# 1812598631/Amos-slam

Measured on AMD Instinct MI355X. Metric: front-end frames/sec (ORB extract+match+mask) at 640x480, higher is better.
Workload: dtype u8 (ORB, gate, matcher) + fp32 (mask network); 1 GPU; configs[2]: 640x480 L8 N1000 full front-end: YOLACT-R50 fp32 mask + ORB detect + gate + describe + match; lanes_per_gpu=2, frames_per_launch=64, width=640, height=480, n_features=1000, n_levels=8, ini_th_fast=20, min_th_fast=7, match=frame k vs k-1, N x N best-2, synthetic_stream_seed=stream = rank, frame k seeded 1000*rank+k (amos-slam_amd/synth.py), parallelism=frames sharded 1 ways, one process per GPU, no data-path collective

## Files before the change

### amos-slam_amd/__init__.py

```python
import ctypes as C
import os

import numpy as np

_HERE = os.path.dirname(os.path.abspath(__file__))
LIB_PATH = os.environ.get("AMOS_FRONTEND_LIB", os.path.join(_HERE, "csrc", "libamos_frontend.so"))

KP_DTYPE = np.dtype([("x", "<f4"), ("y", "<f4"), ("size", "<f4"), ("angle", "<f4"),
                     ("response", "<f4"), ("octave", "<i4"), ("class_id", "<i4")])
BEST2_DTYPE = np.dtype([("best_idx", "<i4"), ("best_dist", "<i4"), ("second_idx", "<i4"),
                        ("second_dist", "<i4")])

TH_HIGH, TH_LOW, HISTO_LENGTH = 100, 50, 30

_v, _i, _z, _f, _d, _q, _u = C.c_void_p, C.c_int, C.c_size_t, C.c_float, C.c_double, C.c_longlong, C.c_uint32
PROTOTYPES = {
    "amos_last_error": (C.c_char_p, ()),
    "amos_device_count": (_i, ()),
    "amos_current_device": (_i, ()),
    "amos_build_variant": (C.c_char_p, ()),
    "amos_orb_create": (_i, (_v, _i, _i, _i, _i, _v, _v)),
    "amos_orb_destroy": (None, (_v,)),
    "amos_orb_geometry_probe": (_i, (_v, _i, _i, _i, _i, _v, _v)),
    "amos_orb_tables": (_i, (_v, _v, _v, _v, _v, _v, _v)),
# ... 53 lines not shown
    "amos_mask_bias_relu_maxpool_device": (_i, (_v, _v, _v, _v, _i, _i, _i, _i)),
    "amos_mask_stem_weight_floats": (_i, ()),
    "amos_mask_stem_weights_device": (_i, (_v, _v, _q, _q, _q, _q, _v)),
    "amos_mask_stem_device": (_i, (_v, _v, _q, _q, _q, _q, _v, _v, _v, _i, _i, _i)),
    "amos_mask_conv_supported": (_i, (_i, _i, _i, _i, _i, _i)),
    "amos_mask_conv_device": (_i, (_v, _v, _v, _v, _v, _v, _i, _i, _i, _i, _i, _i, _i, _i, _i, _i)),
    "amos_mask_conv_workspace_bytes": (_z, (_i, _i, _i, _i, _i, _i, _i, _i, _i)),
    "amos_mask_conv_ws_device": (_i, (_v, _v, _v, _v, _v, _v, _i, _i, _i, _i, _i, _i, _i, _i, _i, _i, _v, _z)),
    "amos_mask_conv_tile_mode": (_i, (_i,)),
    "amos_mask_conv_kernel_name": (_i, (_i, _i, _i, _i, _i, _i, _i, _i, _i, _v, _i)),
    "amos_mask_conv_chain_supported": (_i, (_i, _i, _i, _i, _i, _i, _i)),
    "amos_mask_conv_chain_device": (_i, (_v, _v, _v, _v, _v, _v, _v, _v, _i, _i, _i, _i, _i, _i, _i)),
    "amos_mask_conv1x1_supported": (_i, (_i, _i, _i)),
    "amos_mask_winograd_supported": (_i, (_i, _i)),
    "amos_mask_winograd_weight_floats": (_z, (_i, _i)),
    "amos_mask_winograd_weights_device": (_i, (_v, _v, _v, _i, _i)),
    "amos_mask_winograd_conv_device": (_i, (_v, _v, _v, _v, _v, _v, _i, _i, _i, _i, _i, _i)),
    "amos_mask_winograd24_weight_floats": (_z, (_i, _i)),
    "amos_mask_winograd24_weights_device": (_i, (_v, _v, _v, _i, _i)),
    "amos_mask_winograd24_conv_device": (_i, (_v, _v, _v, _v, _v, _v, _i, _i, _i, _i, _i, _i)),
    "amos_mask_winograd24_conv_layout_device": (_i, (_v, _v, _v, _v, _v, _v, _i, _i, _i, _i, _i, _i, _i, _i)),
    "amos_mask_winograd24_persistent_mode": (_i, (_i,)),
    "amos_mask_winograd24_narrow_mode": (_i, (_i,)),
    "amos_mask_conv1x1_device": (_i, (_v, _v, _v, _v, _v, _v, _i, _i, _i, _i, _i, _i, _i)),
    "amos_mask_bilinear_nhwc_device": (_i, (_v, _v, _v, _i, _i, _i, _i, _i, _i, _f, _f)),
    "amos_mask_bilinear_nhwc_act_device": (_i, (_v, _v, _v, _i, _i, _i, _i, _i, _i, _f, _f, _i)),
    "amos_mask_bilinear_x2_mode": (_i, (_i,)),
    "amos_mask_nms_column_max_device": (_i, (_v, _v, _v, _i, _i)),
    "amos_mask_class_scores_device": (_i, (_v, _v, _v, _i, _i, _i, _f)),
    "amos_mask_person_mask_device": (_i, (_v, _v, _v, _v, _i, _i, _i, _i, _i, _i)),
    "amos_mask_head_outputs_device": (_i, (_v, _v, _v, _v, _v, _v, _i, _i, _i, _i, _i, _i, _i, _i)),
    "amos_mask_head_outputs_scores_device": (_i, (_v, _v, _v, _v, _v, _v, _v, _f, _i, _i, _i, _i, _i, _i, _i, _i)),
    "amos_mask_topk_rows_device": (_i, (_v, _v, _v, _v, _i, _i, _i)),
    "amos_mask_topk_rows_sparse_device": (_i, (_v, _v, _v, _v, _i, _i, _i, _f)),
    "amos_mask_post_workspace_bytes": (_z, (_i, _i, _i, _i, _i, _i)),
    "amos_mask_person_masks_device": (_i, (_v, _v, _v, _v, _v, _v, _i, _i, _i, _i, _i, _i, _i, _i, _v, _z, _v, _v)),
    "amos_mask_person_masks_scores_device": (_i, (_v, _v, _v, _v, _v, _v, _i, _i, _i, _i, _i, _i, _i, _i, _v, _z, _v, _v)),
    "amos_slic_center_count": (_i, (_i, _i, _i, _v, _v)),
    "amos_slic_create": (_i, (_i, _v, _i, _i, _i, _v)),
    "amos_slic_destroy": (None, (_v,)),
    "amos_slic_stream": (_v, (_v,)),
    "amos_slic_run": (_i, (_v, _v, _v, _i, _i, _i, _i, _i, _v, _v, _v)),
    "amos_slic_batch_device": (_i, (_v, _v, _v, _i, _i, _i, _i, _i, _i, _v, _v)),
    "amos_cluster_bgr2lab_batch_device": (_i, (_v, _v, _z, _i, _v)),
    "amos_cluster_kmeans_batch_device": (_i, (_v, _v, _i, _i, _i, _u, _i, _v)),
    "amos_cluster_kmeans": (_i, (_v, _v, _i, _i, _u, _i, _v)),
# ... 432 lines not shown


def mask_conv_supported(cin, cout, kh, kw, stride, pad):
    return lib().amos_mask_conv_supported(cin, cout, kh, kw, stride, pad) == 0


def mask_winograd_supported(cin, cout):
    return lib().amos_mask_winograd_supported(cin, cout) == 0


def mask_winograd_weights(stream_ptr, w_ptr, u_ptr, cin, cout):
    _check(lib().amos_mask_winograd_weights_device(stream_ptr, w_ptr, u_ptr, cin, cout), "amos_mask_winograd_weights_device")


def mask_winograd_conv(stream_ptr, x_ptr, u_ptr, bias_ptr, residual_ptr, y_ptr, batch, h, w, cin, cout, relu):
    _check(lib().amos_mask_winograd_conv_device(stream_ptr, x_ptr, u_ptr, bias_ptr, residual_ptr, y_ptr, batch, h, w, cin, cout, int(relu)),
           "amos_mask_winograd_conv_device")


def mask_winograd24_weights(stream_ptr, w_ptr, u_ptr, cin, cout):
    _check(lib().amos_mask_winograd24_weights_device(stream_ptr, w_ptr, u_ptr, cin, cout), "amos_mask_winograd24_weights_device")


def mask_winograd24_conv(stream_ptr, x_ptr, u_ptr, bias_ptr, residual_ptr, y_ptr, batch, h, w, cin, cout, relu):
    _check(lib().amos_mask_winograd24_conv_device(stream_ptr, x_ptr, u_ptr, bias_ptr, residual_ptr, y_ptr, batch, h, w, cin, cout, int(relu)),
           "amos_mask_winograd24_conv_device")


def mask_winograd24_conv_layout(stream_ptr, x_ptr, u_ptr, bias_ptr, residual_ptr, y_ptr, batch, h, w, cin, cout, relu, in_blocked, out_blocked):
    _check(lib().amos_mask_winograd24_conv_layout_device(stream_ptr, x_ptr, u_ptr, bias_ptr, residual_ptr, y_ptr, batch, h, w, cin, cout, int(relu), int(in_blocked),
                                                         int(out_blocked)), "amos_mask_winograd24_conv_layout_device")


def mask_winograd24_persistent_mode(mode=-2):
    return int(lib().amos_mask_winograd24_persistent_mode(mode))


def mask_winograd24_narrow_mode(mode=-2):
    return int(lib().amos_mask_winograd24_narrow_mode(mode))


def mask_conv_tile_mode(mode=-2):
    return int(lib().amos_mask_conv_tile_mode(mode))


def mask_conv_kernel_name(batch, in_h, in_w, cin, cout, kh, kw, stride, pad):
    buf = C.create_string_buffer(96)
    _check(lib().amos_mask_conv_kernel_name(batch, in_h, in_w, cin, cout, kh, kw, stride, pad, buf, 96), "amos_mask_conv_kernel_name")
    return buf.value.decode()


def mask_conv(stream_ptr, x_ptr, w_ptr, bias_ptr, residual_ptr, y_ptr, batch, in_h, in_w, cin, cout, kh, kw, stride, pad, relu):
    _check(lib().amos_mask_conv_device(stream_ptr, x_ptr, w_ptr, bias_ptr, residual_ptr, y_ptr, batch, in_h, in_w, cin, cout, kh, kw, stride, pad, int(relu)),
           "amos_mask_conv_device")
# ... 318 lines not shown
```

### amos-slam_amd/csrc/amos_mask_post.hip

```cpp
#include <hip/hip_runtime.h>
#include <stdint.h>

#include "../../include/amos_frontend.h"
#include "amos_common.h"

namespace amos {

constexpr int kScoreTile = 64;
__global__ __launch_bounds__(256) void k_class_scores(const float *__restrict__ conf, float *__restrict__ scores, int P, int C1, float thresh)
{
    extern __shared__ float tile[];
    __shared__ float best[kScoreTile];
    const int b = blockIdx.y, p0 = blockIdx.x * kScoreTile, np = min(kScoreTile, P - p0), pitch = C1 + 1;
    const float *src = conf + ((size_t)b * P + p0) * C1;
    for (int e = threadIdx.x; e < np * C1; e += 256) {
        const int r = e / C1, c = e - r * C1;
        tile[r * pitch + c] = src[e];
    }
    __syncthreads();
    if (threadIdx.x < np) {
        const float *row = tile + threadIdx.x * pitch;
        float m = row[1];
        bool nan = m != m;
        for (int c = 2; c < C1; c++) {
// ... 61 lines not shown
            }
        } else {
            for (int i = 0; i < n; i++) {
                if (!flags[b * n + i]) continue;
                const float *m = masks + ((size_t)b * n + i) * ph * pw;
                const float p = m[y0 * pw + x0], r = m[y0 * pw + x1], s2 = m[y1 * pw + x0], u = m[y1 * pw + x1];
                const float v = __fadd_rn(__fmul_rn(hy, __fadd_rn(__fmul_rn(hx, p), __fmul_rn(lx, r))), __fmul_rn(ly, __fadd_rn(__fmul_rn(hx, s2), __fmul_rn(lx, u))));
                count += v > 0.5f ? 1u : 0u;
            }
        }
        out[((size_t)b * H + oy) * W + ox] = (uint8_t)((count * 255u) & 0xffu);
    }
}

constexpr int kHeadCells = 16;
__global__ __launch_bounds__(256) void k_head_outputs(const float *__restrict__ raw, const float *__restrict__ bias, float *__restrict__ loc, float *__restrict__ conf,
                                                     float *__restrict__ coef, int cells, int cpad, int A, int C1, int D, int P, int pOff,
                                                     float *__restrict__ scores, float thresh)
{
    extern __shared__ float sh[];
    const int b = blockIdx.y, c0 = blockIdx.x * kHeadCells, nc = min(kHeadCells, cells - c0);
    const int nLoc = A * 4, nConf = A * C1, nCoef = A * D;
    const float *src = raw + ((size_t)b * cells + c0) * cpad;
    for (int e = threadIdx.x * 4; e < nc * cpad; e += 256 * 4) {
        float4 v = *reinterpret_cast<const float4 *>(src + e);
        const float4 bb = *reinterpret_cast<const float4 *>(bias + e % cpad);
        v.x = __fadd_rn(v.x, bb.x); v.y = __fadd_rn(v.y, bb.y); v.z = __fadd_rn(v.z, bb.z); v.w = __fadd_rn(v.w, bb.w);
        *reinterpret_cast<float4 *>(sh + e) = v;
    }
    __syncthreads();
    __shared__ float sMax[256], sSum[256];
#define AMOS_HEAD_FOREACH(n, body)                                                             \
    {                                                                                          \
        const int stepCell = 256 / (n), stepR = 256 % (n);                                     \
        int cell = (int)threadIdx.x / (n), r = (int)threadIdx.x - cell * (n);                  \
        for (int e = threadIdx.x; e < nc * (n); e += 256) {                                    \
            body;                                                                              \
            cell += stepCell;                                                                  \
            r += stepR;                                                                        \
            if (r >= (n)) { r -= (n); cell++; }                                                \
        }                                                                                      \
    }
    if ((int)threadIdx.x < nc * A) {
        const int cell = threadIdx.x / A, a = threadIdx.x - cell * A;
        const float *v = sh + cell * cpad + nLoc + a * C1;
        float m = v[0];
        for (int c = 1; c < C1; c++) m = fmaxf(m, v[c]);
// ... 852 lines not shown
```

### amos-slam_amd/csrc/amos_winograd24.hip

```cpp
#include <hip/hip_runtime.h>
#include <stdint.h>
#include <stdio.h>
#include <stdlib.h>

#include <algorithm>

#include "../../include/amos_frontend.h"
#include "amos_common.h"

namespace amos {

constexpr int kW24Tiles = 32;
constexpr int kW24Cout = 64;
constexpr int kW24K = 8;
constexpr int kW24Threads = 512;
constexpr int kW24Pos = 24;
#ifndef AMOS_W24_GROUP
#define AMOS_W24_GROUP 16
#endif
constexpr int kW24Group = AMOS_W24_GROUP;
constexpr int kW24StageU = kW24Pos * kW24Cout * kW24K;
constexpr int kW24PosV = kW24Tiles * kW24K;
constexpr int kW24StageV = kW24Pos * kW24PosV;
constexpr int kW24RawCols = 256;
constexpr int kW24RawRow = kW24RawCols * kW24K;
constexpr int kW24StageR = 4 * kW24RawRow;
#ifndef AMOS_W24_XAHEAD
#define AMOS_W24_XAHEAD 1
#endif
constexpr int kW24RawBufs = AMOS_W24_XAHEAD + 1;
constexpr int kW24ExchangeFloats = 8 * 4 * 32 * 32;
constexpr int kW24LoopFloats = 2 * kW24StageV + kW24RawBufs * kW24StageR;
constexpr int kW24LdsFloats = kW24ExchangeFloats > kW24LoopFloats ? kW24ExchangeFloats : kW24LoopFloats;

typedef float f32x16 __attribute__((ext_vector_type(16)));
typedef float f32x4 __attribute__((ext_vector_type(4)));

struct W24Args {
    const float *x, *u, *bias, *res;
    float *y;
    int B, H, W, C, N;
    int tilesX, tilesY, tilesPerImage, totalTiles;
    int mBlocks, nTiles, stages, relu;
    unsigned xBytes;
    unsigned xPixelBytes, xStageBytes;
    int outBlocked;
    int virtualBlocks;
};

__device__ __forceinline__ f32x4 w24_fma(float k, f32x4 a, f32x4 b)
{
    return f32x4{__builtin_fmaf(k, a.x, b.x), __builtin_fmaf(k, a.y, b.y), __builtin_fmaf(k, a.z, b.z), __builtin_fmaf(k, a.w, b.w)};
}

__device__ __host__ __forceinline__ int w24_swz(int row, int half) { return row * 8 + 4 * (half ^ (((row >> 2) ^ (row >> 3)) & 1)); }
__device__ __forceinline__ int w24_raw_unit(int col, int quad) { return (col >> 5) * 64 + (col & 3) * 16 + ((col & 31) >> 2) * 2 + quad; }

__global__ __launch_bounds__(256) void k_winograd24_weights(const float *__restrict__ w, float *__restrict__ u, int cin, int cout)
{
    const int idx = blockIdx.x * 256 + threadIdx.x;
    if (idx >= cin * cout) return;
    const int c = idx % cin, n = idx / cin;
    double g[3][3];
    for (int a = 0; a < 3; a++)
        for (int b = 0; b < 3; b++) g[a][b] = (double)w[((size_t)(n * 3 + a) * 3 + b) * cin + c];
    double t[4][3];
    for (int b = 0; b < 3; b++) {
        t[0][b] = g[0][b];
        t[1][b] = 0.5 * (g[0][b] + g[1][b] + g[2][b]);
        t[2][b] = 0.5 * (g[0][b] - g[1][b] + g[2][b]);
        t[3][b] = g[2][b];
    }
    const int stages = cin / kW24K, nt = n / kW24Cout, nr = n % kW24Cout, s = c / kW24K, k = c % kW24K;
    float *img = u + (size_t)(nt * stages + s) * kW24StageU + (size_t)((nr >> 5) * 64 + (k >> 2) * 32 + (nr & 31)) * 4 + (k & 3);
    for (int a = 0; a < 4; a++) {
        const double t0 = t[a][0], t1 = t[a][1], t2 = t[a][2];
        const double r[6] = {t0 / 4.0, -(t0 + t1 + t2) / 6.0, -(t0 - t1 + t2) / 6.0, t0 / 24.0 + t1 / 12.0 + t2 / 6.0, t0 / 24.0 - t1 / 12.0 + t2 / 6.0, t2};
        for (int b = 0; b < 6; b++) img[(size_t)(a * 6 + b) * 512] = (float)r[b];
    }
}

template <int kHalf, bool kPersist, int kCB>
__device__ __forceinline__ void w24_run(const W24Args &a, float *smem24)
{
    static_assert(kCB == 2 || !kPersist, "the persistent form is written for 64 output channels per work-group");
    constexpr int half = kHalf;
#define AMOS_W24_V(buf) (smem24 + (buf) * kW24StageV)
#define AMOS_W24_R(buf) (smem24 + 2 * kW24StageV + (buf) * kW24StageR)
    const int perXcd = (a.mBlocks + 7) >> 3;
    auto decode = [&](int id, int &mbOut, int &ntOut) -> bool {
        const int xcd = id & 7, seq = id >> 3;
        const int per = kW24Group * a.nTiles, grp = seq / per, in = seq - grp * per;
        const int mbLocal = grp * kW24Group + in % kW24Group;
        ntOut = in / kW24Group;
        mbOut = xcd * perXcd + mbLocal;
        return mbLocal < perXcd && mbOut < a.mBlocks;
    };
    auto next_valid = [&](int id, int &mbOut, int &ntOut) -> int {
        for (; id < a.virtualBlocks; id += (int)gridDim.x)
            if (decode(id, mbOut, ntOut)) return id;
        return -1;
    };
    int mb = 0, nt = 0;
    int id = kPersist ? next_valid((int)blockIdx.x, mb, nt) : (decode((int)blockIdx.x, mb, nt) ? (int)blockIdx.x : -1);
    if (id < 0) return;
    const int t = threadIdx.x, lane = t & 63, wave = __builtin_amdgcn_readfirstlane(t >> 6);

    const int quad = lane & 1, tl = lane >> 1, prow = wave >> 1;
    const int col = 32 * wave + 4 * ((lane >> 1) & 7) + (lane >> 4);
    auto geometry = [&](int mbi, int (&xo)[4], int &cbase) {
        const int T0 = mbi * kW24Tiles, nT = min(kW24Tiles, a.totalTiles - T0);
        int b = T0 / a.tilesPerImage, rem = T0 - b * a.tilesPerImage, ty = rem / a.tilesX, tx = rem - ty * a.tilesX;
        cbase = 0;
#pragma unroll
        for (int r = 0; r < 4; r++) xo[r] = (int)a.xBytes;
        for (int t0 = 0, cb = 0; t0 < nT;) {
            const int n = min(a.tilesX - tx, nT - t0);
            if (col >= cb && col < cb + 4 * n + 2) {
                const int lc = col - cb, tloc = min(lc >> 2, n - 1), ix = 4 * (tx + tloc) - 1 + (lc - 4 * tloc);
#pragma unroll
                for (int r = 0; r < 4; r++) {
                    const int iy = 2 * ty - 1 + r;
                    if ((unsigned)iy < (unsigned)a.H && (unsigned)ix < (unsigned)a.W)
                        xo[r] = (int)((unsigned)b * (unsigned)(a.H * a.W) * (unsigned)a.C * 4u + (unsigned)(iy * a.W + ix) * a.xPixelBytes + 16u * quad);
                }
            }
            if (tl >= t0 && tl < t0 + n) cbase = cb + 4 * (tl - t0);
// ... 360 lines not shown
        }
    }
    if (!kPersist || !haveNext) break;
    id = idN; mb = mbN; nt = ntN;
#pragma unroll
    for (int r = 0; r < 4; r++) xoff[r] = xoffN[r];
    colBase = colBaseN;
    usrc = usrcN;
    AMOS_W24_SET_RSRC()
    AMOS_W24_ZERO_ACC()
    asm volatile("s_waitcnt vmcnt(0) lgkmcnt(0)\n\ts_barrier" ::: "memory");
    AMOS_W24_TRANSFORM(0, 0);
    asm volatile("s_waitcnt lgkmcnt(0)\n\ts_barrier" ::: "memory");
    AMOS_W24_LDFRAG(fa0, 0, 0);
    AMOS_W24_FETCH_X(2, 0);
    }
#undef AMOS_W24_V
#undef AMOS_W24_R
}

__global__ __launch_bounds__(kW24Threads) __attribute__((amdgpu_waves_per_eu(2, 2))) void k_winograd24_conv(const W24Args a)
{
    extern __shared__ __align__(16) float smem24[];
    if (__builtin_amdgcn_readfirstlane(threadIdx.x >> 6) & 1) w24_run<1, false, 2>(a, smem24);
    else w24_run<0, false, 2>(a, smem24);
}

__global__ __launch_bounds__(kW24Threads) __attribute__((amdgpu_waves_per_eu(2, 2))) void k_winograd24_conv_n32(const W24Args a)
{
    extern __shared__ __align__(16) float smem24[];
    if (__builtin_amdgcn_readfirstlane(threadIdx.x >> 6) & 1) w24_run<1, false, 1>(a, smem24);
    else w24_run<0, false, 1>(a, smem24);
}

__global__ __launch_bounds__(kW24Threads) __attribute__((amdgpu_waves_per_eu(2, 2))) void k_winograd24_conv_persistent(const W24Args a)
{
    extern __shared__ __align__(16) float smem24[];
    if (__builtin_amdgcn_readfirstlane(threadIdx.x >> 6) & 1) w24_run<1, true, 2>(a, smem24);
    else w24_run<0, true, 2>(a, smem24);
}

const char *w24_variant_tag()
{
    return ""
#ifdef AMOS_W24_EXP_NOX
        " AMOS_W24_EXP_NOX"
#endif
#ifdef AMOS_W24_EXP_NOU
        " AMOS_W24_EXP_NOU"
#endif
#ifdef AMOS_W24_EXP_NOT
        " AMOS_W24_EXP_NOT"
#endif
#ifdef AMOS_W24_EXP_NOBAR
        " AMOS_W24_EXP_NOBAR"
#endif
#ifdef AMOS_W24_EXP_NOEPI
        " AMOS_W24_EXP_NOEPI"
#endif
        ;
}

// ... 1 lines not shown

using namespace amos;

static int g_w24_persist = -2;
static int w24_persist_mode()
{
    if (g_w24_persist == -2) {
        const char *env = getenv("AMOS_W24_PERSIST");
        g_w24_persist = env && (env[0] == '0' || env[0] == '1') ? env[0] - '0' : -1;
    }
    return g_w24_persist;
}

static int g_w24_narrow = -2;
static int w24_narrow_mode()
{
    if (g_w24_narrow == -2) {
        const char *env = getenv("AMOS_W24_NARROW");
        g_w24_narrow = env && (env[0] == '0' || env[0] == '1') ? env[0] - '0' : -1;
    }
    return g_w24_narrow;
}

extern "C" {

int amos_mask_winograd24_narrow_mode(int mode)
{
    const int before = w24_narrow_mode();
    if (mode >= -1 && mode <= 1) g_w24_narrow = mode;
    return before;
}

int amos_mask_winograd24_persistent_mode(int mode)
{
    const int before = w24_persist_mode();
    if (mode >= -1 && mode <= 1) g_w24_persist = mode;
    return before;
}

size_t amos_mask_winograd24_weight_floats(int cin, int cout)
{
    return amos_mask_winograd_supported(cin, cout) == AMOS_OK ? (size_t)kW24Pos * cin * cout : 0;
}

int amos_mask_winograd24_weights_device(void *stream, const float *d_w, float *d_u, int cin, int cout)
{
    if (!d_w || !d_u || amos_mask_winograd_supported(cin, cout) != AMOS_OK) {
        set_error("amos_mask_winograd24_weights_device: invalid argument (cin %% 16 == 0, cin >= 32, cout %% 64 == 0)");
        return AMOS_ERR_INVALID;
    }
    hipLaunchKernelGGL(k_winograd24_weights, dim3((unsigned)((cin * cout + 255) / 256)), dim3(256), 0, (hipStream_t)stream, d_w, d_u, cin, cout);
    AMOS_HIP_CHECK(hipGetLastError());
    return AMOS_OK;
}

int amos_mask_winograd24_conv_device(void *stream, const float *d_x, const float *d_u, const float *d_bias, const float *d_residual, float *d_y,
                                     int batch, int h, int w, int cin, int cout, int relu)
{
    return amos_mask_winograd24_conv_layout_device(stream, d_x, d_u, d_bias, d_residual, d_y, batch, h, w, cin, cout, relu, 0, 0);
}

int amos_mask_winograd24_conv_layout_device(void *stream, const float *d_x, const float *d_u, const float *d_bias, const float *d_residual, float *d_y,
                                            int batch, int h, int w, int cin, int cout, int relu, int in_blocked, int out_blocked)
{
    const long long xBytes = (long long)batch * h * w * cin * 4;
    if (!d_x || !d_u || !d_y || batch < 1 || h < 1 || w < 1 || amos_mask_winograd_supported(cin, cout) != AMOS_OK || xBytes > 0x7fffffffLL - 4096 ||
        ((uintptr_t)d_x | (uintptr_t)d_u | (uintptr_t)d_y | (uintptr_t)d_bias | (uintptr_t)d_residual) % 16 != 0) {
        set_error("amos_mask_winograd24_conv_device: invalid argument (cin %% 16 == 0, cin >= 32, cout %% 64 == 0, input below 2 GiB, 16-byte aligned channels-last tensors)");
        return AMOS_ERR_INVALID;
    }
    static DeviceOnce ldsAttr, ldsAttrP, ldsAttrN;
    const size_t lds = (size_t)kW24LdsFloats * sizeof(float);
    AMOS_HIP_CHECK(set_max_dynamic_lds(ldsAttr, reinterpret_cast<const void *>(k_winograd24_conv), (int)lds, (hipStream_t)stream));
    W24Args a;
    a.x = d_x; a.u = d_u; a.bias = d_bias; a.res = d_residual; a.y = d_y;
    a.B = batch; a.H = h; a.W = w; a.C = cin; a.N = cout;
    a.tilesX = (w + 3) / 4; a.tilesY = (h + 1) / 2;
    a.tilesPerImage = a.tilesX * a.tilesY;
    a.totalTiles = batch * a.tilesPerImage;
    a.mBlocks = (a.totalTiles + kW24Tiles - 1) / kW24Tiles;
    const int narrowMode = w24_narrow_mode();
    const bool narrow = narrowMode >= 0 ? narrowMode != 0 : (long long)a.mBlocks * (cout / kW24Cout) <= 100;
    a.nTiles = cout / (narrow ? 32 : kW24Cout);
    a.stages = cin / kW24K;
    a.relu = relu;
    a.xBytes = (unsigned)xBytes;
    a.xPixelBytes = in_blocked ? 32u : (unsigned)cin * 4u;
    a.xStageBytes = in_blocked ? (unsigned)(h * w) * 32u : 32u;
    a.outBlocked = out_blocked ? 1 : 0;
    const int perXcd = (a.mBlocks + 7) / 8, groups = (perXcd + kW24Group - 1) / kW24Group;
    a.virtualBlocks = groups * kW24Group * a.nTiles * 8;
    const dim3 block(kW24Threads);
    const int forced = w24_persist_mode();
    static int cus = 0;
    if (cus == 0) {
        int dev = 0;
        hipDeviceProp_t prop;
        if (hipGetDevice(&dev) == hipSuccess && hipGetDeviceProperties(&prop, dev) == hipSuccess) cus = prop.multiProcessorCount / 8 * 8;
        if (cus < 8) cus = 256;
    }
    const bool persist = forced == 1 && a.virtualBlocks > cus && !narrow;
    if (persist) {
        AMOS_HIP_CHECK(set_max_dynamic_lds(ldsAttrP, reinterpret_cast<const void *>(k_winograd24_conv_persistent), (int)lds, (hipStream_t)stream));
        hipLaunchKernelGGL(k_winograd24_conv_persistent, dim3((unsigned)std::min(cus, a.virtualBlocks)), block, lds, (hipStream_t)stream, a);
    } else if (narrow) {
        AMOS_HIP_CHECK(set_max_dynamic_lds(ldsAttrN, reinterpret_cast<const void *>(k_winograd24_conv_n32), (int)lds, (hipStream_t)stream));
        hipLaunchKernelGGL(k_winograd24_conv_n32, dim3((unsigned)a.virtualBlocks), block, lds, (hipStream_t)stream, a);
    } else {
        hipLaunchKernelGGL(k_winograd24_conv, dim3((unsigned)a.virtualBlocks), block, lds, (hipStream_t)stream, a);
    }
    AMOS_HIP_CHECK(hipGetLastError());
    return AMOS_OK;
}

}
```

### amos-slam_amd/mask/net.py

```python
import math
import os

import torch
import torch.nn as nn
import torch.nn.functional as F

NUM_CLASSES = 81
MASK_DIM = 32
FPN_FEATURES = 256
CONF_THRESH = 0.05
MAX_SIZE = 550
PRED_SCALES = (24, 48, 96, 192, 384)
ASPECT_RATIOS = (1.0, 0.5, 2.0)


def _gemm_conv(conv, x):
    k = conv.kernel_size
    if k[0] != k[1] or conv.padding[0] != conv.padding[1] or conv.dilation != (1, 1) or conv.groups != 1 or conv.stride[0] != conv.stride[1]:
        return False
    from .. import mask_conv_supported
    if not mask_conv_supported(conv.in_channels, conv.out_channels, k[0], k[1], conv.stride[0], conv.padding[0]):
        return False
    s = conv.stride[0]
    m = x.shape[0] * ((x.shape[2] + 2 * conv.padding[0] - k[0]) // s + 1) * ((x.shape[3] + 2 * conv.padding[1] - k[1]) // s + 1)
# ... 111 lines not shown

def prepare_stem_weight(module):
    n = 0
    for m in module.modules():
        if isinstance(m, ResNet50Trunk) and _stem_eligible(m.conv1) and stem_kernel_enabled():
            _stem_weight(m.conv1)
            n += 1
    return n


class Blocked:
    __slots__ = ("data", "shape")
    is_cuda = True
    dtype = torch.float32

    def __init__(self, data, shape):
        self.data, self.shape = data, tuple(shape)

    @property
    def device(self):
        return self.data.device


def _winograd24_layout(conv, x, bias, residual, relu, out_blocked):
    from .. import mask_winograd24_conv_layout
    in_blocked = isinstance(x, Blocked)
    b, _, h, w = x.shape
    dev = x.device
    if out_blocked:
        y = Blocked(torch.empty((b, conv.out_channels // 8, h, w, 8), device=dev, dtype=torch.float32), (b, conv.out_channels, h, w))
    else:
        y = torch.empty((b, conv.out_channels, h, w), device=dev, dtype=torch.float32, memory_format=torch.channels_last)
    mask_winograd24_conv_layout(torch.cuda.current_stream(dev).cuda_stream, (x.data if in_blocked else x).data_ptr(), _winograd_weight(conv).data_ptr(),
                                bias.data_ptr() if bias is not None else None, residual.data_ptr() if residual is not None else None,
                                (y.data if out_blocked else y).data_ptr(), b, h, w, conv.in_channels, conv.out_channels, relu, in_blocked, out_blocked)
    return y


def blocked_chain_for(p3_in, convs_69, convs_138):
    if os.environ.get("AMOS_MASK_BLOCKED_CHAIN", "1") == "0" or winograd_family() != "24" or torch.is_autocast_enabled():
        return False
    if not (p3_in.is_cuda and p3_in.dtype == torch.float32 and p3_in.shape[0] >= 8 and p3_in.is_contiguous(memory_format=torch.channels_last)):
        return False
    b, _, h, w = p3_in.shape
    ok = all(c.bias is not None and c.weight.dtype == torch.float32 and c.in_channels % 8 == 0 and c.out_channels % 8 == 0 and
             winograd_rule(c.in_channels, c.out_channels, c.kernel_size, c.stride, c.padding, c.dilation, c.groups, b, h, w) for c in convs_69)
    return ok and all(c.bias is not None and c.weight.dtype == torch.float32 and
                      winograd_rule(c.in_channels, c.out_channels, c.kernel_size, c.stride, c.padding, c.dilation, c.groups, b, 2 * h, 2 * w) for c in convs_138)


def conv_raw(conv, x):
    cl = torch.channels_last
    if isinstance(x, Blocked):
        return _winograd24_layout(conv, x, None, None, False, False)
    if x.is_cuda and x.dtype == torch.float32 and not torch.is_autocast_enabled() and x.is_contiguous(memory_format=cl) and conv.weight.dtype == torch.float32:
        if _winograd_conv(conv, x):
            b, _, h, w = x.shape
            y = torch.empty((b, conv.out_channels, h, w), device=x.device, dtype=torch.float32, memory_format=cl)
            _winograd_fns()[3](torch.cuda.current_stream(x.device).cuda_stream, x.data_ptr(), _winograd_weight(conv).data_ptr(), None, None, y.data_ptr(),
                               b, h, w, conv.in_channels, conv.out_channels, False)
            return y
    return F.conv2d(x, conv.weight, None, conv.stride, conv.padding, conv.dilation, conv.groups)


def conv_bias_act(conv, x, relu, residual=None, out_blocked=False):
    if isinstance(x, Blocked) or out_blocked:
        if residual is not None:
            raise ValueError("conv_bias_act: no residual in the channel-blocked chain")
        return _winograd24_layout(conv, x, conv.bias, None, relu, out_blocked)
    if x.is_cuda and conv.bias is not None and x.dtype == torch.float32 and not torch.is_autocast_enabled():
        cl = torch.channels_last
        if _winograd_conv(conv, x) and x.is_contiguous(memory_format=cl) and conv.weight.dtype == torch.float32 and (residual is None or (
                residual.dtype == torch.float32 and residual.is_contiguous(memory_format=cl))):
            b, _, h, w = x.shape
            y = torch.empty((b, conv.out_channels, h, w), device=x.device, dtype=torch.float32, memory_format=cl)
            if residual is not None and residual.shape != y.shape:
                raise ValueError("conv_bias_act: residual shape %s, output shape %s" % (tuple(residual.shape), tuple(y.shape)))
            _winograd_fns()[3](torch.cuda.current_stream(x.device).cuda_stream, x.data_ptr(), _winograd_weight(conv).data_ptr(), conv.bias.data_ptr(),
                               residual.data_ptr() if residual is not None else None, y.data_ptr(), b, h, w, conv.in_channels, conv.out_channels, relu)
            return y
        if _gemm_conv(conv, x) and x.is_contiguous(memory_format=cl) and conv.weight.dtype == torch.float32 and (
                conv.weight.is_contiguous(memory_format=cl) or (conv.kernel_size == (1, 1) and conv.weight.is_contiguous())) and (residual is None or (
                residual.dtype == torch.float32 and residual.is_contiguous(memory_format=cl))):
# ... 285 lines not shown
            n = sum(l.out_channels for l in layers)
            pad = (-n) % 64
            merged = nn.Conv2d(FPN_FEATURES, n + pad, 3, padding=1).to(device=self.bbox_layer.weight.device, dtype=self.bbox_layer.weight.dtype)
            with torch.no_grad():
                merged.weight.zero_()
                merged.bias.zero_()
                merged.weight[:n].copy_(torch.cat([l.weight for l in layers], 0))
                merged.bias[:n].copy_(torch.cat([l.bias for l in layers], 0))
            object.__setattr__(self, "merged", merged.requires_grad_(False))
        return self

    def fused_applies(self, x0):
        merged = getattr(self, "merged", None)
        return not (merged is None or not x0.is_cuda or x0.dtype != torch.float32 or torch.is_autocast_enabled() or os.environ.get("AMOS_MASK_FUSED_HEAD", "1") == "0")

    def fused_outputs(self, pyramid, n_priors, br=None, out=None, scores=None):
        x0 = pyramid[0]
        if not self.fused_applies(x0):
            return None
        merged = self.merged
        from .. import mask_head_outputs_scores
        b, dev = x0.shape[0], x0.device
        n_anchor = self.bbox_layer.out_channels // 4
        if out is None:
            if br is not None:
                raise ValueError("fused_outputs: with side streams the caller allocates the outputs")
            out = self.alloc_outputs(b, n_priors, dev)
        loc, conf, coef = out
        offs, off = [], 0
        for x in pyramid:
            offs.append(off)
            off += x.shape[2] * x.shape[3] * n_anchor
        if off != n_priors:
            raise ValueError("fused_outputs: %d priors written, %d expected" % (off, n_priors))

        def level(i):
            x = pyramid[i]
            u = conv_bias_act(self.upfeature[0], x, True, out_blocked=isinstance(x, Blocked))
            raw = conv_raw(merged, u)
            if not raw.is_contiguous(memory_format=torch.channels_last):
                raw = raw.contiguous(memory_format=torch.channels_last)
            cells = raw.shape[2] * raw.shape[3]
            mask_head_outputs_scores(torch.cuda.current_stream(dev).cuda_stream, raw.data_ptr(), merged.bias.data_ptr(), loc.data_ptr(),
                                     conf.data_ptr() if conf is not None else None, coef.data_ptr(), scores.data_ptr() if scores is not None else None,
                                     CONF_THRESH, b, cells, raw.shape[1], n_anchor, NUM_CLASSES, MASK_DIM, n_priors, offs[i])

        if br is not None and len(pyramid) == 5:
            with br.side(2 if len(br.streams) >= 3 else None):
                level(0)
            with br.side(1, fork=False):
                level(1)
            with br.side(0, fork=False):
                for i in (2, 3, 4):
                    level(i)
        else:
            for i in range(len(pyramid)):
                level(i)
        return loc, conf, coef

    def alloc_outputs(self, b, n_priors, dev, conf=True):
        return (torch.empty((b, n_priors, 4), dtype=torch.float32, device=dev),
                torch.empty((b, n_priors, NUM_CLASSES), dtype=torch.float32, device=dev) if conf else None,
# ... 138 lines not shown
```

### include/amos_frontend.h

```cpp
#ifndef AMOS_FRONTEND_H
#define AMOS_FRONTEND_H

#include <stddef.h>
#include <stdint.h>

#ifdef __cplusplus
extern "C" {
#endif

#define AMOS_OK 0
#define AMOS_ERR_INVALID (-1)
#define AMOS_ERR_DEVICE (-2)
#define AMOS_ERR_CAPACITY (-3)
#define AMOS_ERR_STATE (-4)

#define AMOS_EDGE_THRESHOLD 19
#define AMOS_MAX_LEVELS 16
#define AMOS_FRAME_GRID_ROWS 48
#define AMOS_FRAME_GRID_COLS 64
#define AMOS_TH_HIGH 100
#define AMOS_TH_LOW 50
#define AMOS_HISTO_LENGTH 30

typedef struct amos_keypoint {
// ... 190 lines not shown
                             int batch, int in_h, int in_w, int cin, int cout, int kh, int kw, int stride, int pad, int relu,
                             void *d_workspace, size_t workspace_bytes);
int amos_mask_conv_tile_mode(int mode);
int amos_mask_conv_kernel_name(int batch, int in_h, int in_w, int cin, int cout, int kh, int kw, int stride, int pad, char *name,
                               int name_len);
int amos_mask_conv_chain_supported(int batch, int in_h, int in_w, int cin, int planes, int cout, int stride);
int amos_mask_conv_chain_device(void *stream, const float *d_x, const float *d_wd, const float *d_bd, const float *d_yc, const float *d_w3,
                                const float *d_b3, float *d_y, int batch, int in_h, int in_w, int cin, int planes, int cout, int stride);
int amos_mask_conv1x1_supported(int cin, int cout, int stride);

int amos_mask_winograd_supported(int cin, int cout);
size_t amos_mask_winograd_weight_floats(int cin, int cout);
int amos_mask_winograd_weights_device(void *stream, const float *d_w, float *d_u, int cin, int cout);
int amos_mask_winograd_conv_device(void *stream, const float *d_x, const float *d_u, const float *d_bias, const float *d_residual,
                                   float *d_y, int batch, int h, int w, int cin, int cout, int relu);
size_t amos_mask_winograd24_weight_floats(int cin, int cout);
int amos_mask_winograd24_weights_device(void *stream, const float *d_w, float *d_u, int cin, int cout);
int amos_mask_winograd24_conv_device(void *stream, const float *d_x, const float *d_u, const float *d_bias, const float *d_residual,
                                     float *d_y, int batch, int h, int w, int cin, int cout, int relu);
int amos_mask_winograd24_conv_layout_device(void *stream, const float *d_x, const float *d_u, const float *d_bias, const float *d_residual,
                                            float *d_y, int batch, int h, int w, int cin, int cout, int relu, int in_blocked, int out_blocked);
int amos_mask_winograd24_persistent_mode(int mode);
int amos_mask_winograd24_narrow_mode(int mode);
int amos_mask_conv1x1_device(void *stream, const float *d_x, const float *d_w, const float *d_bias, const float *d_residual,
                             float *d_y, int batch, int in_h, int in_w, int cin, int cout, int stride, int relu);

int amos_mask_bilinear_nhwc_device(void *stream, const float *d_x, float *d_y, int n, int in_h, int in_w, int out_h,
                                   int out_w, int channels, float scale_h, float scale_w);

int amos_mask_bilinear_nhwc_act_device(void *stream, const float *d_x, float *d_y, int n, int in_h, int in_w, int out_h,
                                       int out_w, int channels, float scale_h, float scale_w, int relu);

int amos_mask_bilinear_x2_mode(int mode);

int amos_mask_nms_column_max_device(void *stream, const float *d_boxes, float *d_out, int n_lists, int k);

int amos_mask_class_scores_device(void *stream, const float *d_conf, float *d_scores, int batch, int n_priors,
                                  int n_classes_with_background, float threshold);

int amos_mask_person_mask_device(void *stream, const float *d_masks, const uint8_t *d_flags, uint8_t *d_out, int batch, int n_det,
                                 int mask_h, int mask_w, int out_h, int out_w);

int amos_mask_head_outputs_device(void *stream, const float *d_raw, const float *d_bias, float *d_loc, float *d_conf, float *d_coef,
                                  int batch, int cells, int channels_padded, int anchors, int n_classes_with_background, int mask_dim,
                                  int n_priors_total, int prior_offset);
int amos_mask_head_outputs_scores_device(void *stream, const float *d_raw, const float *d_bias, float *d_loc, float *d_conf, float *d_coef, float *d_scores,
// ... 175 lines not shown
```

Before: 1618 frames/s.

## Skip dead padded head channels and split ragged Winograd grids into half tiles

Adds a cout_live path to the Winograd F(2,4) conv so the merged prediction-head conv computes only the channels the head actually reads, rounded up to 32. A ragged final tile runs as a 32-channel half tile. A mixed kernel and a cost-model launch planner are also added: groups that fill whole rounds of CUs run as 64-channel tiles, and the leftover groups run as pairs of 32-channel half tiles to cut tail-round imbalance. The head-output kernel now skips padded channels. Costs are more kernel variants, a host-side id-limit search with a small cache, and an environment-tunable half-tile cost heuristic that may mispredict.

New measurement: 1618 frames/s (median of 2 runs). Within noise of the previous version (+0.0%).

```diff
diff --git a/amos-slam_amd/__init__.py b/amos-slam_amd/__init__.py
--- a/amos-slam_amd/__init__.py
+++ b/amos-slam_amd/__init__.py
@@ -99,6 +99,10 @@
     "amos_mask_winograd24_conv_layout_device": (_i, (_v, _v, _v, _v, _v, _v, _i, _i, _i, _i, _i, _i, _i, _i)),
     "amos_mask_winograd24_persistent_mode": (_i, (_i,)),
     "amos_mask_winograd24_narrow_mode": (_i, (_i,)),
+    "amos_mask_winograd24_conv_live_device": (_i, (_v, _v, _v, _v, _v, _v, _i, _i, _i, _i, _i, _i, _i, _i, _i)),
+    "amos_mask_launch_plan_mode": (_i, (_i,)),
+    "amos_mask_winograd24_mixed_mode": (_i, (_i,)),
+    "amos_mask_winograd24_plan": (_i, (_i, _i, _i, _i, _i, _v, _v)),
     "amos_mask_conv1x1_device": (_i, (_v, _v, _v, _v, _v, _v, _i, _i, _i, _i, _i, _i, _i)),
     "amos_mask_bilinear_nhwc_device": (_i, (_v, _v, _v, _i, _i, _i, _i, _i, _i, _f, _f)),
     "amos_mask_bilinear_nhwc_act_device": (_i, (_v, _v, _v, _i, _i, _i, _i, _i, _i, _f, _f, _i)),
@@ -577,14 +581,38 @@
     _check(lib().amos_mask_winograd24_weights_device(stream_ptr, w_ptr, u_ptr, cin, cout), "amos_mask_winograd24_weights_device")
 
 
-def mask_winograd24_conv(stream_ptr, x_ptr, u_ptr, bias_ptr, residual_ptr, y_ptr, batch, h, w, cin, cout, relu):
+def mask_winograd24_conv(stream_ptr, x_ptr, u_ptr, bias_ptr, residual_ptr, y_ptr, batch, h, w, cin, cout, relu, cout_live=None):
+    if cout_live is not None:
+        return mask_winograd24_conv_live(stream_ptr, x_ptr, u_ptr, bias_ptr, residual_ptr, y_ptr, batch, h, w, cin, cout, cout_live, relu, False, False)
     _check(lib().amos_mask_winograd24_conv_device(stream_ptr, x_ptr, u_ptr, bias_ptr, residual_ptr, y_ptr, batch, h, w, cin, cout, int(relu)),
            "amos_mask_winograd24_conv_device")
 
 
-def mask_winograd24_conv_layout(stream_ptr, x_ptr, u_ptr, bias_ptr, residual_ptr, y_ptr, batch, h, w, cin, cout, relu, in_blocked, out_blocked):
+def mask_winograd24_conv_layout(stream_ptr, x_ptr, u_ptr, bias_ptr, residual_ptr, y_ptr, batch, h, w, cin, cout, relu, in_blocked, out_blocked, cout_live=None):
+    if cout_live is not None:
+        return mask_winograd24_conv_live(stream_ptr, x_ptr, u_ptr, bias_ptr, residual_ptr, y_ptr, batch, h, w, cin, cout, cout_live, relu, in_blocked, out_blocked)
     _check(lib().amos_mask_winograd24_conv_layout_device(stream_ptr, x_ptr, u_ptr, bias_ptr, residual_ptr, y_ptr, batch, h, w, cin, cout, int(relu), int(in_blocked),
                                                          int(out_blocked)), "amos_mask_winograd24_conv_layout_device")
+
+
+def mask_winograd24_conv_live(stream_ptr, x_ptr, u_ptr, bias_ptr, residual_ptr, y_ptr, batch, h, w, cin, cout, cout_live, relu, in_blocked, out_blocked):
+    _check(lib().amos_mask_winograd24_conv_live_device(stream_ptr, x_ptr, u_ptr, bias_ptr, residual_ptr, y_ptr, batch, h, w, cin, cout, cout_live, int(relu),
+                                                       int(in_blocked), int(out_blocked)), "amos_mask_winograd24_conv_live_device")
+
+
+def mask_launch_plan_mode(mode=-2):
+    return int(lib().amos_mask_launch_plan_mode(mode))
+
+
+def mask_winograd24_mixed_mode(n_large=-2):
+    return int(lib().amos_mask_winograd24_mixed_mode(n_large))
+
+
+def mask_winograd24_plan(batch, h, w, cout, cus):
+    import ctypes
+    a, b = ctypes.c_longlong(0), ctypes.c_longlong(0)
+    _check(lib().amos_mask_winograd24_plan(batch, h, w, cout, cus, ctypes.byref(a), ctypes.byref(b)), "amos_mask_winograd24_plan")
+    return a.value, b.value
 
 
 def mask_winograd24_persistent_mode(mode=-2):
diff --git a/amos-slam_amd/csrc/amos_launch_plan.h b/amos-slam_amd/csrc/amos_launch_plan.h
--- /dev/null
+++ b/amos-slam_amd/csrc/amos_launch_plan.h
@@ -0,0 +1,43 @@
+#ifndef AMOS_LAUNCH_PLAN_H
+#define AMOS_LAUNCH_PLAN_H
+
+namespace amos {
+
+struct LaunchPlan {
+    long long n_large;
+    long long n_half;
+    double cost;
+    double single_cost;
+};
+
+constexpr int kPlanMinRounds = 2;
+
+inline long long plan_rounds(long long groups, int slots) { return (groups + slots - 1) / slots; }
+
+inline double plan_cost(long long n_large, long long n_half, int slots, double half_cost)
+{
+    return (double)plan_rounds(n_large, slots) + half_cost * (double)plan_rounds(n_half, slots);
+}
+
+inline LaunchPlan plan_launch(long long groups, int slots, double half_cost, bool single_half)
+{
+    if (groups < 0) groups = 0;
+    if (slots < 1) slots = 1;
+    LaunchPlan single;
+    single.n_large = single_half ? 0 : groups;
+    single.n_half = single_half ? 2 * groups : 0;
+    single.cost = single.single_cost = plan_cost(single.n_large, single.n_half, slots, half_cost);
+    if (single_half) return single;
+    const long long whole = groups / slots * slots;
+    if (whole < (long long)kPlanMinRounds * slots || whole == groups) return single;
+    LaunchPlan mixed;
+    mixed.n_large = whole;
+    mixed.n_half = 2 * (groups - whole);
+    mixed.cost = plan_cost(mixed.n_large, mixed.n_half, slots, half_cost);
+    mixed.single_cost = single.cost;
+    return mixed.cost < single.cost ? mixed : single;
+}
+
+}
+
+#endif
diff --git a/amos-slam_amd/csrc/amos_mask_post.hip b/amos-slam_amd/csrc/amos_mask_post.hip
--- a/amos-slam_amd/csrc/amos_mask_post.hip
+++ b/amos-slam_amd/csrc/amos_mask_post.hip
@@ -107,7 +107,9 @@
     const int b = blockIdx.y, c0 = blockIdx.x * kHeadCells, nc = min(kHeadCells, cells - c0);
     const int nLoc = A * 4, nConf = A * C1, nCoef = A * D;
     const float *src = raw + ((size_t)b * cells + c0) * cpad;
+    const int nLive = nLoc + nConf + nCoef;
     for (int e = threadIdx.x * 4; e < nc * cpad; e += 256 * 4) {
+        if (e % cpad >= nLive) continue;
         float4 v = *reinterpret_cast<const float4 *>(src + e);
         const float4 bb = *reinterpret_cast<const float4 *>(bias + e % cpad);
         v.x = __fadd_rn(v.x, bb.x); v.y = __fadd_rn(v.y, bb.y); v.z = __fadd_rn(v.z, bb.z); v.w = __fadd_rn(v.w, bb.w);
diff --git a/amos-slam_amd/csrc/amos_winograd24.hip b/amos-slam_amd/csrc/amos_winograd24.hip
--- a/amos-slam_amd/csrc/amos_winograd24.hip
+++ b/amos-slam_amd/csrc/amos_winograd24.hip
@@ -7,6 +7,7 @@
 
 #include "../../include/amos_frontend.h"
 #include "amos_common.h"
+#include "amos_launch_plan.h"
 
 namespace amos {
 
@@ -46,7 +47,19 @@
     unsigned xPixelBytes, xStageBytes;
     int outBlocked;
     int virtualBlocks;
+    int nLarge, raggedN;
 };
+
+__host__ __device__ __forceinline__ bool w24_decode(int mBlocks, int nTiles, int id, int &mbOut, int &ntOut)
+{
+    const int perXcd = (mBlocks + 7) >> 3;
+    const int xcd = id & 7, seq = id >> 3;
+    const int per = kW24Group * nTiles, grp = seq / per, in = seq - grp * per;
+    const int mbLocal = grp * kW24Group + in % kW24Group;
+    ntOut = in / kW24Group;
+    mbOut = xcd * perXcd + mbLocal;
+    return mbLocal < perXcd && mbOut < mBlocks;
+}
 
 __device__ __forceinline__ f32x4 w24_fma(float k, f32x4 a, f32x4 b)
 {
@@ -81,28 +94,20 @@
 }
 
 template <int kHalf, bool kPersist, int kCB>
-__device__ __forceinline__ void w24_run(const W24Args &a, float *smem24)
+__device__ __forceinline__ void w24_run(const W24Args &a, float *smem24, int mbFirst, int ntFirst)
 {
     static_assert(kCB == 2 || !kPersist, "the persistent form is written for 64 output channels per work-group");
     constexpr int half = kHalf;
 #define AMOS_W24_V(buf) (smem24 + (buf) * kW24StageV)
 #define AMOS_W24_R(buf) (smem24 + 2 * kW24StageV + (buf) * kW24StageR)
-    const int perXcd = (a.mBlocks + 7) >> 3;
-    auto decode = [&](int id, int &mbOut, int &ntOut) -> bool {
-        const int xcd = id & 7, seq = id >> 3;
-        const int per = kW24Group * a.nTiles, grp = seq / per, in = seq - grp * per;
-        const int mbLocal = grp * kW24Group + in % kW24Group;
-        ntOut = in / kW24Group;
-        mbOut = xcd * perXcd + mbLocal;
-        return mbLocal < perXcd && mbOut < a.mBlocks;
-    };
+    auto decode = [&](int id, int &mbOut, int &ntOut) -> bool { return w24_decode(a.mBlocks, a.nTiles, id, mbOut, ntOut); };
     auto next_valid = [&](int id, int &mbOut, int &ntOut) -> int {
         for (; id < a.virtualBlocks; id += (int)gridDim.x)
             if (decode(id, mbOut, ntOut)) return id;
         return -1;
     };
-    int mb = 0, nt = 0;
-    int id = kPersist ? next_valid((int)blockIdx.x, mb, nt) : (decode((int)blockIdx.x, mb, nt) ? (int)blockIdx.x : -1);
+    int mb = mbFirst, nt = ntFirst;
+    int id = kPersist ? next_valid((int)blockIdx.x, mb, nt) : (int)blockIdx.x;
     if (id < 0) return;
     const int t = threadIdx.x, lane = t & 63, wave = __builtin_amdgcn_readfirstlane(t >> 6);
 
@@ -509,22 +514,53 @@
 __global__ __launch_bounds__(kW24Threads) __attribute__((amdgpu_waves_per_eu(2, 2))) void k_winograd24_conv(const W24Args a)
 {
     extern __shared__ __align__(16) float smem24[];
-    if (__builtin_amdgcn_readfirstlane(threadIdx.x >> 6) & 1) w24_run<1, false, 2>(a, smem24);
-    else w24_run<0, false, 2>(a, smem24);
+    int mb, nt;
+    if (!w24_decode(a.mBlocks, a.nTiles, (int)blockIdx.x, mb, nt)) return;
+    if (__builtin_amdgcn_readfirstlane(threadIdx.x >> 6) & 1) w24_run<1, false, 2>(a, smem24, mb, nt);
+    else w24_run<0, false, 2>(a, smem24, mb, nt);
 }
 
 __global__ __launch_bounds__(kW24Threads) __attribute__((amdgpu_waves_per_eu(2, 2))) void k_winograd24_conv_n32(const W24Args a)
 {
     extern __shared__ __align__(16) float smem24[];
-    if (__builtin_amdgcn_readfirstlane(threadIdx.x >> 6) & 1) w24_run<1, false, 1>(a, smem24);
-    else w24_run<0, false, 1>(a, smem24);
+    int mb, nt;
+    if (!w24_decode(a.mBlocks, a.nTiles, (int)blockIdx.x, mb, nt)) return;
+    if (__builtin_amdgcn_readfirstlane(threadIdx.x >> 6) & 1) w24_run<1, false, 1>(a, smem24, mb, nt);
+    else w24_run<0, false, 1>(a, smem24, mb, nt);
+}
+
+__global__ __launch_bounds__(kW24Threads) __attribute__((amdgpu_waves_per_eu(2, 2))) void k_winograd24_conv_mixed(const W24Args a)
+{
+    extern __shared__ __align__(16) float smem24[];
+    const int b = (int)blockIdx.x;
+    bool half = b >= a.nLarge;
+    int id = b, h = 0;
+    if (half) {
+        const int r = b - a.nLarge;
+        h = (r >> 3) & 1;
+        id = a.nLarge + (r >> 4) * 8 + (r & 7);
+    }
+    int mb, nt;
+    if (id >= a.virtualBlocks || !w24_decode(a.mBlocks, a.nTiles, id, mb, nt)) return;
+    if (a.raggedN && nt == a.nTiles - 1) {
+        if (h) return;
+        half = true;
+    }
+    const bool odd = __builtin_amdgcn_readfirstlane(threadIdx.x >> 6) & 1;
+    if (half) {
+        if (odd) w24_run<1, false, 1>(a, smem24, mb, 2 * nt + h);
+        else w24_run<0, false, 1>(a, smem24, mb, 2 * nt + h);
+    } else {
+        if (odd) w24_run<1, false, 2>(a, smem24, mb, nt);
+        else w24_run<0, false, 2>(a, smem24, mb, nt);
+    }
 }
 
 __global__ __launch_bounds__(kW24Threads) __attribute__((amdgpu_waves_per_eu(2, 2))) void k_winograd24_conv_persistent(const W24Args a)
 {
     extern __shared__ __align__(16) float smem24[];
-    if (__builtin_amdgcn_readfirstlane(threadIdx.x >> 6) & 1) w24_run<1, true, 2>(a, smem24);
-    else w24_run<0, true, 2>(a, smem24);
+    if (__builtin_amdgcn_readfirstlane(threadIdx.x >> 6) & 1) w24_run<1, true, 2>(a, smem24, 0, 0);
+    else w24_run<0, true, 2>(a, smem24, 0, 0);
 }
 
 const char *w24_variant_tag()
@@ -572,7 +608,67 @@
     return g_w24_narrow;
 }
 
+static int g_launch_plan = -2;
+static int launch_plan_mode()
+{
+    if (g_launch_plan == -2) {
+        const char *env = getenv("AMOS_LAUNCH_PLAN");
+        g_launch_plan = env && env[0] == '0' ? 0 : 1;
+    }
+    return g_launch_plan;
+}
+
+static int g_w24_mixed = -1;
+
+static double w24_half_cost()
+{
+    static const double c = getenv("AMOS_W24_HALF_COST") ? atof(getenv("AMOS_W24_HALF_COST")) : 0.75;
+    return c;
+}
+
+static int w24_id_limit(int mBlocks, int nTiles, int virtualBlocks, long long groups)
+{
+    if (groups >= (long long)mBlocks * nTiles) return virtualBlocks;
+    struct Key { int mBlocks, nTiles; long long groups; int limit; };
+    thread_local Key cache[8] = {};
+    thread_local int next = 0;
+    for (const Key &k : cache)
+        if (k.mBlocks == mBlocks && k.nTiles == nTiles && k.groups == groups) return k.limit;
+    int id = 0, mb, nt;
+    for (long long seen = 0; id < virtualBlocks && seen < groups; id++) seen += w24_decode(mBlocks, nTiles, id, mb, nt) ? 1 : 0;
+    cache[next] = Key{mBlocks, nTiles, groups, id};
+    next = (next + 1) & 7;
+    return id;
+}
+
 extern "C" {
+
+int amos_mask_launch_plan_mode(int mode)
+{
+    const int before = launch_plan_mode();
+    if (mode == 0 || mode == 1) g_launch_plan = mode;
+    return before;
+}
+
+int amos_mask_winograd24_mixed_mode(int n_large)
+{
+    const int before = g_w24_mixed;
+    if (n_large >= -1) g_w24_mixed = n_large;
+    return before;
+}
+
+int amos_mask_winograd24_plan(int batch, int h, int w, int cout, int cus, long long *n_large, long long *n_half)
+{
+    if (batch < 1 || h < 1 || w < 1 || cout < 64 || cout % 64 != 0 || cus < 1 || !n_large || !n_half) {
+        set_error("amos_mask_winograd24_plan: invalid argument");
+        return AMOS_ERR_INVALID;
+    }
+    const long long mBlocks = ((long long)batch * ((w + 3) / 4) * ((h + 1) / 2) + kW24Tiles - 1) / kW24Tiles, groups = mBlocks * (cout / kW24Cout);
+    const LaunchPlan plan = plan_launch(groups, cus, w24_half_cost(), groups <= 100);
+    *n_large = plan.n_large;
+    *n_half = plan.n_half;
+    return AMOS_OK;
+}
 
 int amos_mask_winograd24_narrow_mode(int mode)
 {
@@ -607,12 +703,22 @@
 int amos_mask_winograd24_conv_device(void *stream, const float *d_x, const float *d_u, const float *d_bias, const float *d_residual, float *d_y,
                                      int batch, int h, int w, int cin, int cout, int relu)
 {
-    return amos_mask_winograd24_conv_layout_device(stream, d_x, d_u, d_bias, d_residual, d_y, batch, h, w, cin, cout, relu, 0, 0);
+    return amos_mask_winograd24_conv_live_device(stream, d_x, d_u, d_bias, d_residual, d_y, batch, h, w, cin, cout, cout, relu, 0, 0);
 }
 
 int amos_mask_winograd24_conv_layout_device(void *stream, const float *d_x, const float *d_u, const float *d_bias, const float *d_residual, float *d_y,
                                             int batch, int h, int w, int cin, int cout, int relu, int in_blocked, int out_blocked)
 {
+    return amos_mask_winograd24_conv_live_device(stream, d_x, d_u, d_bias, d_residual, d_y, batch, h, w, cin, cout, cout, relu, in_blocked, out_blocked);
+}
+
+int amos_mask_winograd24_conv_live_device(void *stream, const float *d_x, const float *d_u, const float *d_bias, const float *d_residual, float *d_y,
+                                          int batch, int h, int w, int cin, int cout, int cout_live, int relu, int in_blocked, int out_blocked)
+{
+    if (cout_live < 32 || cout_live > cout || cout_live % 32 != 0 || cout - cout_live >= kW24Cout) {
+        set_error("amos_mask_winograd24_conv_live_device: cout_live must be a multiple of 32 within the last 64 channels of cout");
+        return AMOS_ERR_INVALID;
+    }
     const long long xBytes = (long long)batch * h * w * cin * 4;
     if (!d_x || !d_u || !d_y || batch < 1 || h < 1 || w < 1 || amos_mask_winograd_supported(cin, cout) != AMOS_OK || xBytes > 0x7fffffffLL - 4096 ||
         ((uintptr_t)d_x | (uintptr_t)d_u | (uintptr_t)d_y | (uintptr_t)d_bias | (uintptr_t)d_residual) % 16 != 0) {
@@ -631,7 +737,11 @@
     a.mBlocks = (a.totalTiles + kW24Tiles - 1) / kW24Tiles;
     const int narrowMode = w24_narrow_mode();
     const bool narrow = narrowMode >= 0 ? narrowMode != 0 : (long long)a.mBlocks * (cout / kW24Cout) <= 100;
-    a.nTiles = cout / (narrow ? 32 : kW24Cout);
+    const bool planned = launch_plan_mode() != 0;
+    const int live = planned && !(narrowMode < 0 && narrow) ? cout_live : cout;
+    const bool ragged = live % kW24Cout != 0;
+    a.nTiles = narrow ? live / 32 : (live + kW24Cout - 1) / kW24Cout;
+    a.raggedN = ragged ? 1 : 0;
     a.stages = cin / kW24K;
     a.relu = relu;
     a.xBytes = (unsigned)xBytes;
@@ -649,8 +759,21 @@
         if (hipGetDevice(&dev) == hipSuccess && hipGetDeviceProperties(&prop, dev) == hipSuccess) cus = prop.multiProcessorCount / 8 * 8;
         if (cus < 8) cus = 256;
     }
-    const bool persist = forced == 1 && a.virtualBlocks > cus && !narrow;
-    if (persist) {
+    const bool persist = forced == 1 && a.virtualBlocks > cus && !narrow && !ragged;
+    const long long allGroups = (long long)a.mBlocks * a.nTiles;
+    long long largeGroups = allGroups;
+    if (!narrow && !persist) {
+        if (g_w24_mixed >= 0) largeGroups = std::min<long long>(g_w24_mixed, allGroups);
+        else if (planned && narrowMode < 0 && !ragged) largeGroups = plan_launch(allGroups, cus, w24_half_cost(), false).n_large;
+    }
+    a.nLarge = a.virtualBlocks;
+    static DeviceOnce ldsAttrM;
+    if (!narrow && !persist && (ragged || largeGroups < allGroups)) {
+        a.nLarge = w24_id_limit(a.mBlocks, a.nTiles, a.virtualBlocks, largeGroups);
+        const int rest = a.virtualBlocks - a.nLarge;
+        AMOS_HIP_CHECK(set_max_dynamic_lds(ldsAttrM, reinterpret_cast<const void *>(k_winograd24_conv_mixed), (int)lds, (hipStream_t)stream));
+        hipLaunchKernelGGL(k_winograd24_conv_mixed, dim3((unsigned)(a.nLarge + (rest + 7) / 8 * 16)), block, lds, (hipStream_t)stream, a);
+    } else if (persist) {
         AMOS_HIP_CHECK(set_max_dynamic_lds(ldsAttrP, reinterpret_cast<const void *>(k_winograd24_conv_persistent), (int)lds, (hipStream_t)stream));
         hipLaunchKernelGGL(k_winograd24_conv_persistent, dim3((unsigned)std::min(cus, a.virtualBlocks)), block, lds, (hipStream_t)stream, a);
     } else if (narrow) {
diff --git a/amos-slam_amd/mask/net.py b/amos-slam_amd/mask/net.py
--- a/amos-slam_amd/mask/net.py
+++ b/amos-slam_amd/mask/net.py
@@ -157,7 +157,7 @@
         return self.data.device
 
 
-def _winograd24_layout(conv, x, bias, residual, relu, out_blocked):
+def _winograd24_layout(conv, x, bias, residual, relu, out_blocked, live_channels=None):
     from .. import mask_winograd24_conv_layout
     in_blocked = isinstance(x, Blocked)
     b, _, h, w = x.shape
@@ -168,7 +168,8 @@
         y = torch.empty((b, conv.out_channels, h, w), device=dev, dtype=torch.float32, memory_format=torch.channels_last)
     mask_winograd24_conv_layout(torch.cuda.current_stream(dev).cuda_stream, (x.data if in_blocked else x).data_ptr(), _winograd_weight(conv).data_ptr(),
                                 bias.data_ptr() if bias is not None else None, residual.data_ptr() if residual is not None else None,
-                                (y.data if out_blocked else y).data_ptr(), b, h, w, conv.in_channels, conv.out_channels, relu, in_blocked, out_blocked)
+                                (y.data if out_blocked else y).data_ptr(), b, h, w, conv.in_channels, conv.out_channels, relu, in_blocked, out_blocked,
+                                *(() if live_channels is None else (live_channels,)))
     return y
 
 
@@ -184,16 +185,17 @@
                       winograd_rule(c.in_channels, c.out_channels, c.kernel_size, c.stride, c.padding, c.dilation, c.groups, b, 2 * h, 2 * w) for c in convs_138)
 
 
-def conv_raw(conv, x):
+def conv_raw(conv, x, live_channels=None):
     cl = torch.channels_last
     if isinstance(x, Blocked):
-        return _winograd24_layout(conv, x, None, None, False, False)
+        return _winograd24_layout(conv, x, None, None, False, False, live_channels)
     if x.is_cuda and x.dtype == torch.float32 and not torch.is_autocast_enabled() and x.is_contiguous(memory_format=cl) and conv.weight.dtype == torch.float32:
         if _winograd_conv(conv, x):
             b, _, h, w = x.shape
             y = torch.empty((b, conv.out_channels, h, w), device=x.device, dtype=torch.float32, memory_format=cl)
+            live = (live_channels,) if live_channels is not None and winograd_family() == "24" else ()
             _winograd_fns()[3](torch.cuda.current_stream(x.device).cuda_stream, x.data_ptr(), _winograd_weight(conv).data_ptr(), None, None, y.data_ptr(),
-                               b, h, w, conv.in_channels, conv.out_channels, False)
+                               b, h, w, conv.in_channels, conv.out_channels, False, *live)
             return y
     return F.conv2d(x, conv.weight, None, conv.stride, conv.padding, conv.dilation, conv.groups)
 
@@ -525,6 +527,7 @@
         from .. import mask_head_outputs_scores
         b, dev = x0.shape[0], x0.device
         n_anchor = self.bbox_layer.out_channels // 4
+        n_live = self.bbox_layer.out_channels + self.conf_layer.out_channels + self.mask_layer.out_channels
         if out is None:
             if br is not None:
                 raise ValueError("fused_outputs: with side streams the caller allocates the outputs")
@@ -540,7 +543,7 @@
         def level(i):
             x = pyramid[i]
             u = conv_bias_act(self.upfeature[0], x, True, out_blocked=isinstance(x, Blocked))
-            raw = conv_raw(merged, u)
+            raw = conv_raw(merged, u, live_channels=min(merged.out_channels, (n_live + 31) // 32 * 32))
             if not raw.is_contiguous(memory_format=torch.channels_last):
                 raw = raw.contiguous(memory_format=torch.channels_last)
             cells = raw.shape[2] * raw.shape[3]
diff --git a/include/amos_frontend.h b/include/amos_frontend.h
--- a/include/amos_frontend.h
+++ b/include/amos_frontend.h
@@ -236,6 +236,12 @@
                                             float *d_y, int batch, int h, int w, int cin, int cout, int relu, int in_blocked, int out_blocked);
 int amos_mask_winograd24_persistent_mode(int mode);
 int amos_mask_winograd24_narrow_mode(int mode);
+int amos_mask_winograd24_conv_live_device(void *stream, const float *d_x, const float *d_u, const float *d_bias, const float *d_residual,
+                                          float *d_y, int batch, int h, int w, int cin, int cout, int cout_live, int relu, int in_blocked,
+                                          int out_blocked);
+int amos_mask_launch_plan_mode(int mode);
+int amos_mask_winograd24_mixed_mode(int n_large);
+int amos_mask_winograd24_plan(int batch, int h, int w, int cout, int cus, long long *n_large, long long *n_half);
 int amos_mask_conv1x1_device(void *stream, const float *d_x, const float *d_w, const float *d_bias, const float *d_residual,
                              float *d_y, int batch, int in_h, int in_w, int cin, int cout, int stride, int relu);
 
```
